# barathanaslan/whisper-ipa

Hardware: AMD Instinct MI355X
Metric: audio-seconds/sec transcribed (whisper-small, 30s clips) (higher is better)
Workload: dtype bf16

## Files before the change

include/wipa.h:

```cpp
#ifndef WIPA_H
#define WIPA_H
#include <stddef.h>
#include <stdint.h>
#ifdef __cplusplus
extern "C" {
#endif

typedef void* wipa_stream_t;

enum { WIPA_F32 = 0, WIPA_BF16 = 1, WIPA_FP8_E4M3 = 2  };
enum { WIPA_OK = 0, WIPA_ERR_ARG = -1, WIPA_ERR_HIP = -2, WIPA_ERR_STATE = -3 };

#define WIPA_N_SAMPLES 480000
#define WIPA_N_FRAMES 3000
#define WIPA_N_FFT 400
#define WIPA_HOP 160
#define WIPA_HEAD_DIM 64

int wipa_version(void);
const char* wipa_last_error(void);

int wipa_stream_create(wipa_stream_t* out);
int wipa_stream_create_cu_limited(int n_cus, wipa_stream_t* out);
int wipa_stream_destroy(wipa_stream_t s);
// ... 127 lines not shown
    const int32_t* pos;
    float* slabs;
    int64_t kv_batch_stride, slab_stride;
    int32_t B, d, H, dtype;
    float eps, qk_scale;
} wipa_self_block_desc;
int wipa_decode_self_block(const wipa_self_block_desc* d, wipa_stream_t s);
typedef struct wipa_cross_block_desc {
    const float* x_in;
    float* x_out;
    const float* slabs;
    const float* bias_o;
    const float* ln_w;
    const float* ln_b;
    const void* wq;
    const float* bq;
    const void* kv;
    void* out;
    int64_t slab_stride;
    int32_t n_slabs, B, d, H, Tk, dtype;
    float eps, qk_scale;
    int32_t cross_splits;
} wipa_cross_block_desc;
int wipa_decode_cross_block(const wipa_cross_block_desc* d, wipa_stream_t s);

int wipa_cross_absorbed_splits(int want, int Tk);
int wipa_cross_absorbed_resident_groups_for(int B, int d, int Tk, int n_splits, int64_t budget_bytes);
int wipa_cross_absorbed_resident_groups(int B, int d, int Tk, int n_splits);
size_t wipa_cross_absorbed_scratch_bytes(int B, int d, int Tk);
int wipa_cross_absorbed_init(int d);
int wipa_cross_absorbed_attention(const void* q, int64_t q_row_stride, const void* wkT, const void* xa, const void* wv, const float* bv,
                                  void* out, int64_t out_row_stride, void* scratch, size_t scratch_bytes, int B, int H, int d, int Tk,
                                  float k_scale, int n_splits, wipa_stream_t s);
int wipa_decode_cross_absorbed_block(const wipa_cross_block_desc* c, const void* wkT, const void* wv, const float* bv, void* scratch,
                                     size_t scratch_bytes, wipa_stream_t s);
int wipa_decode_cross_absorbed_block_out(const wipa_cross_block_desc* c, const void* wkT, const void* wv, const float* bv, const void* wo,
                                         const float* bo, float* slabs_out, int64_t slab_stride, void* scratch, size_t scratch_bytes,
                                         wipa_stream_t s);
int wipa_cross_absorbed_stream(const void* xa, void* scratch, size_t scratch_bytes, int B, int H, int d, int Tk, int n_splits,
                               wipa_stream_t s);

int wipa_greedy_step(const float* logits, int64_t ldl, int B, int V, const float* mask_first,
                     const float* mask_always, int32_t* tokens, int64_t ld_tok, const int32_t* pos_dev, int n_init,
                     int eot, float* sum_logprobs, int32_t* not_done, wipa_stream_t s);
int wipa_add_i32(int32_t* p, int32_t v, wipa_stream_t s);
int wipa_greedy_step_embed(const float* logits, int64_t ldl, int B, int V, const float* mask_first, const float* mask_always,
                           int32_t* tokens, int64_t ld_tok, int32_t* pos_dev, int64_t* posd_dev, int32_t* done_counter, int n_init,
                           int eot, float* sum_logprobs, int32_t* not_done, const void* tok_emb, int emb_dtype,
                           const float* emb_scale, const float* pos_emb, int n_ctx, float* x, const float* ln_w, const float* ln_b,
                           void* y, int y_dtype, int D, float eps, wipa_stream_t s);
#define WIPA_GREEDY_PARTS 2048
int wipa_logits_greedy_supported(int B, int V, int d, int dtype);
size_t wipa_logits_greedy_partials_bytes(int B);
int wipa_logits_greedy(const void* x, int64_t ldx, const void* w, int64_t ldw, float* logits, int64_t ldl, int B, int V, int d,
                       const float* mask_first, const float* mask_always, const int32_t* pos_dev, int n_init, float* partials,
                       size_t partials_bytes, wipa_stream_t s);
int wipa_greedy_step_embed_partials(const float* partials, int n_parts, int B, int32_t* tokens, int64_t ld_tok, int32_t* pos_dev,
                                    int64_t* posd_dev, int32_t* done_counter, int n_init, int eot, float* sum_logprobs,
                                    int32_t* not_done, const void* tok_emb, int emb_dtype, const float* emb_scale, const float* pos_emb,
                                    int n_ctx, float* x, const float* ln_w, const float* ln_b, void* y, int y_dtype, int D, float eps,
                                    wipa_stream_t s);
int wipa_embed_layernorm(const int32_t* tokens, int64_t ld_tok, int B, const int32_t* pos_dev, const void* tok_emb, int emb_dtype,
                         const float* emb_scale, const float* pos_emb, int n_ctx, float* x, const float* ln_w, const float* ln_b,
                         void* y, int y_dtype, int D, float eps, wipa_stream_t s);

typedef struct wipa_bpe wipa_bpe;
// ... 95 lines not shown
```

whisper_ipa_amd/_lib.py:

```python
from __future__ import annotations

import ctypes as C
import os
import threading

_HERE = os.path.dirname(os.path.abspath(__file__))
LIB_PATH = os.path.join(_HERE, "libwipa.so")

WIPA_F32, WIPA_BF16, WIPA_FP8_E4M3 = 0, 1, 2
GREEDY_PARTS = 2048
RESAMPLE_TILE = 512
ENC_GLOBAL, ENC_PER_LAYER = 7, 14
DEC_GLOBAL, DEC_PER_LAYER, DEC_FP8_PER_LAYER = 4, 20, 6
GEMM_DISPATCH = ("tile128", "tile256", "tile384", "tile384n", "tile256p", "skinny", "skinny_fp8", "skinny_ln", "kmajor", "split_k",
                 "tile_fp8", "tile_fp8_384")
ENC_FP8_PER_LAYER = 8
DEC_ABSORBED_PER_LAYER = 1

c_void_p, c_int, c_int64, c_size_t, c_float = C.c_void_p, C.c_int, C.c_int64, C.c_size_t, C.c_float


class GemmDesc(C.Structure):
    _fields_ = [
        ("A", c_void_p), ("W", c_void_p), ("C", c_void_p), ("bias", c_void_p), ("residual", c_void_p),
# ... 73 lines not shown
    "wipa_stream_destroy": (c_int, [c_void_p]),
    "wipa_resample_pad": (c_int, [c_void_p, c_size_t, c_void_p, _P(PcmClipDesc), c_int, c_void_p, c_size_t, c_void_p, c_void_p]),
    "wipa_logmel_tables_bytes": (c_size_t, [c_int]),
    "wipa_logmel_init": (c_int, [c_void_p, c_int, c_void_p]),
    "wipa_logmel_workspace_bytes": (c_size_t, [c_int, c_int]),
    "wipa_logmel": (c_int, [c_void_p, c_int, c_int, c_void_p, c_void_p, c_int, c_void_p, c_size_t, c_void_p]),
    "wipa_mel_pad_cast": (c_int, [c_void_p, c_int, c_int, c_void_p, c_int, c_void_p]),
    "wipa_gemm": (c_int, [_P(GemmDesc), c_void_p]),
    "wipa_gemm_dispatch_counts": (c_int, [_P(c_int64), c_int, c_int]),
    "wipa_layernorm": (c_int, [c_void_p, c_int, c_int64, c_void_p, c_int, c_int64, c_void_p, c_void_p, c_int, c_int,
                               c_float, c_void_p]),
    "wipa_layernorm_fp8": (c_int, [c_void_p, c_int64, c_void_p, c_int64, c_void_p, c_void_p, c_void_p, c_int, c_int, c_float, c_void_p]),
    "wipa_rowquant_fp8": (c_int, [c_void_p, c_int, c_int64, c_void_p, c_int64, c_void_p, c_int, c_int, c_void_p]),
    "wipa_add_slabs_layernorm": (c_int, [c_void_p, c_int64, c_void_p, c_int, c_int64, c_void_p, c_int, c_int64, c_void_p,
                                         c_void_p, c_int, c_int, c_float, c_void_p]),
    "wipa_embed_tokens": (c_int, [c_void_p, c_int64, c_int, c_int, c_int, c_void_p, c_void_p, c_int, c_void_p, c_void_p, c_void_p,
                                  c_int, c_void_p]),
    "wipa_attention": (c_int, [_P(AttnDesc), c_void_p]),
    "wipa_flash_attn_enc_f32": (c_int, [c_void_p, c_int64, c_void_p, c_int64, c_void_p, c_int64, c_void_p, c_int64, c_int, c_int,
                                       c_int, c_int, c_void_p]),
    "wipa_flash_attn_enc_bf16": (c_int, [c_void_p, c_int64, c_void_p, c_int64, c_void_p, c_int64, c_int, c_int, c_int,
                                         c_void_p]),
    "wipa_decode_attn": (c_int, [_P(AttnDesc), c_void_p]),
    "wipa_decode_cross_attn": (c_int, [c_void_p, c_void_p, c_void_p, c_int, c_int, c_int, c_int, c_void_p]),
    "wipa_decode_self_block": (c_int, [_P(SelfBlockDesc), c_void_p]),
    "wipa_decode_cross_block": (c_int, [_P(CrossBlockDesc), c_void_p]),
    "wipa_cross_absorbed_splits": (c_int, [c_int, c_int]),
    "wipa_cross_absorbed_resident_groups_for": (c_int, [c_int, c_int, c_int, c_int, c_int64]),
    "wipa_cross_absorbed_resident_groups": (c_int, [c_int, c_int, c_int, c_int]),
    "wipa_cross_absorbed_scratch_bytes": (c_size_t, [c_int, c_int, c_int]),
    "wipa_cross_absorbed_init": (c_int, [c_int]),
    "wipa_cross_absorbed_attention": (c_int, [c_void_p, c_int64, c_void_p, c_void_p, c_void_p, c_void_p, c_void_p, c_int64, c_void_p, c_size_t,
                                              c_int, c_int, c_int, c_int, c_float, c_int, c_void_p]),
    "wipa_cross_absorbed_stream": (c_int, [c_void_p, c_void_p, c_size_t, c_int, c_int, c_int, c_int, c_int, c_void_p]),
    "wipa_decode_cross_absorbed_block": (c_int, [_P(CrossBlockDesc), c_void_p, c_void_p, c_void_p, c_void_p, c_size_t, c_void_p]),
    "wipa_decode_cross_absorbed_block_out": (c_int, [_P(CrossBlockDesc), c_void_p, c_void_p, c_void_p, c_void_p, c_void_p, c_void_p, c_int64,
                                                     c_void_p, c_size_t, c_void_p]),
    "wipa_greedy_step": (c_int, [c_void_p, c_int64, c_int, c_int, c_void_p, c_void_p, c_void_p, c_int64, c_void_p, c_int,
                                 c_int, c_void_p, c_void_p, c_void_p]),
    "wipa_add_i32": (c_int, [c_void_p, C.c_int32, c_void_p]),
    "wipa_greedy_step_embed": (c_int, [c_void_p, c_int64, c_int, c_int, c_void_p, c_void_p, c_void_p, c_int64, c_void_p, c_void_p, c_void_p,
                                       c_int, c_int, c_void_p, c_void_p, c_void_p, c_int, c_void_p, c_void_p, c_int, c_void_p, c_void_p,
                                       c_void_p, c_void_p, c_int, c_int, c_float, c_void_p]),
    "wipa_logits_greedy_supported": (c_int, [c_int, c_int, c_int, c_int]),
    "wipa_logits_greedy_partials_bytes": (c_size_t, [c_int]),
    "wipa_logits_greedy": (c_int, [c_void_p, c_int64, c_void_p, c_int64, c_void_p, c_int64, c_int, c_int, c_int, c_void_p, c_void_p, c_void_p,
                                   c_int, c_void_p, c_size_t, c_void_p]),
    "wipa_greedy_step_embed_partials": (c_int, [c_void_p, c_int, c_int, c_void_p, c_int64, c_void_p, c_void_p, c_void_p, c_int, c_int, c_void_p,
                                                c_void_p, c_void_p, c_int, c_void_p, c_void_p, c_int, c_void_p, c_void_p, c_void_p, c_void_p,
                                                c_int, c_int, c_float, c_void_p]),
    "wipa_embed_layernorm": (c_int, [c_void_p, c_int64, c_int, c_void_p, c_void_p, c_int, c_void_p, c_void_p, c_int, c_void_p, c_void_p,
                                     c_void_p, c_void_p, c_int, c_int, c_float, c_void_p]),
    "wipa_bpe_create": (c_void_p, [c_void_p, c_void_p, c_void_p, c_int]),
    "wipa_bpe_free": (None, [c_void_p]),
    "wipa_bpe_encode_piece": (c_int, [c_void_p, C.c_char_p, c_int, c_void_p, c_int]),
    "wipa_bpe_decode": (c_int, [c_void_p, c_void_p, c_int, c_void_p, c_int]),
    "wipa_build_token_batch": (c_int, [c_void_p, c_void_p, c_int, c_void_p, c_int, C.c_int32, c_void_p, c_int64]),
    "wipa_profile_begin": (c_int, [c_void_p]),
    "wipa_profile_end": (c_int, [_P(c_float), _P(c_int)]),
    "wipa_encoder_workspace_bytes": (c_size_t, [_P(ModelCfg), c_int]),
    "wipa_encoder_forward": (c_int, [_P(ModelCfg), _P(c_void_p), c_void_p, c_void_p, c_void_p, c_size_t, c_int, c_void_p]),
    "wipa_decoder_layout": (c_int, [_P(ModelCfg), c_int, _P(DecLayout)]),
    "wipa_decoder_set_audio": (c_int, [_P(ModelCfg), _P(c_void_p), c_void_p, c_void_p, c_size_t, c_int, c_void_p]),
    "wipa_decoder_begin": (c_int, [_P(ModelCfg), c_void_p, c_size_t, c_int, _P(C.c_int32), c_int, c_void_p]),
    "wipa_decoder_run": (c_int, [_P(ModelCfg), _P(c_void_p), c_void_p, c_size_t, c_int, c_int, c_int, c_void_p, c_void_p, c_int,
                                 c_int, c_void_p]),
# ... 58 lines not shown
```

whisper_ipa_amd/csrc/cross_absorbed.hip:

```cpp
#include <cstdlib>
#include <mutex>
#include <type_traits>

#include "attn_stream.h"
#include "wipa_common.h"

namespace {

constexpr int FT = 32;
constexpr long long XA_RESIDENT_MB_SHARED = 16;
constexpr long long XA_RESIDENT_MB_LONE = -1;
typedef __attribute__((address_space(3))) void* lds_ptr_a;
typedef int v2i32 __attribute__((ext_vector_type(2)));

struct AbsParams {
    const __bf16* qp;
    const __bf16* xa;
    float* part_m;
    float* part_l;
    float* part_o;
    int Tk, n_splits, tiles_per_split, H;
    int resident_groups;
};

constexpr int POLICY_DEFAULT = 0, POLICY_NT = 2;

__device__ __forceinline__ int swz(int row) { return (row & 7) << 1; }

template <int D>
struct AbsCfg {
    static constexpr int NW = 4;
    static constexpr int ROWB = D * 2;
    static constexpr int TILE = FT * ROWB;
    static constexpr int SX = NW * 2 * 64 * 4 * (int)sizeof(float);
    static constexpr int NBUF = (3 * TILE + SX <= 160 * 1024) ? 3 : 2;
    static constexpr int SMEM = NBUF * TILE + SX;
};

template <int D>
__global__ __launch_bounds__(512, 1) void cross_absorbed_kernel(AbsParams p) {
    typedef AbsCfg<D> X;
    constexpr int NW = X::NW, ROWB = X::ROWB, TILE = X::TILE, NBUF = X::NBUF;
    constexpr int NDMA = TILE / 1024 / NW;
    constexpr int KS = D / NW / 32;
    constexpr int CT = D / NW / 16;
    static_assert(D % (32 * NW) == 0 && TILE % (1024 * NW) == 0, "width");
    extern __shared__ __attribute__((aligned(1024))) char smem[];
    float* sx = reinterpret_cast<float*>(smem + NBUF * TILE);
    const int tid = threadIdx.x, lane = tid & 63;
    const int wave = __builtin_amdgcn_readfirstlane(tid >> 6);
    const int l15 = lane & 15, g = lane >> 4;
    const int split = blockIdx.x, b = blockIdx.y;
    const int tile0 = split * p.tiles_per_split;
    const int n_tiles_total = (p.Tk + FT - 1) / FT;
    const int nt = max(0, min(p.tiles_per_split, n_tiles_total - tile0));
    const __bf16* xb = p.xa + (int64_t)b * p.Tk * D;

    bf16x8 qf[KS];
    {
        const __bf16* qr = p.qp + ((int64_t)b * 16 + l15) * D + wave * (D / NW) + 8 * g;
#pragma unroll
        for (int ks = 0; ks < KS; ++ks) qf[ks] = *reinterpret_cast<const bf16x8*>(qr + 32 * ks);
    }
    const __amdgpu_buffer_rsrc_t rX = __builtin_amdgcn_make_buffer_rsrc((void*)xb, 0, 0x7fffffff, 0x00020000);
    int drow[NDMA], dch[NDMA];
#pragma unroll
    for (int i = 0; i < NDMA; ++i) {
        const int off = 1024 * (NDMA * wave + i) + 16 * lane;
        drow[i] = off / ROWB;
        dch[i] = ((off % ROWB) >> 4) ^ swz(off / ROWB);
    }
    const int res_tiles = p.resident_groups / 2;
    auto stage_as = [&](auto policy, int t, int buf) {
        constexpr int AUX = decltype(policy)::value;
        const int f0 = (tile0 + t) * FT;
#pragma unroll
        for (int i = 0; i < NDMA; ++i) {
            const int voff = min(f0 + drow[i], p.Tk - 1) * ROWB + dch[i] * 16;
            __builtin_amdgcn_raw_ptr_buffer_load_lds(rX, (lds_ptr_a)(smem + buf * TILE + 1024 * (NDMA * wave + i)), 16, voff, 0, 0, AUX);
        }
    };
    auto stage = [&](int t, int buf) {
        if (t < res_tiles) stage_as(std::integral_constant<int, POLICY_DEFAULT>{}, t, buf);
        else stage_as(std::integral_constant<int, POLICY_NT>{}, t, buf);
    };
    auto wait_dma = [&](bool one_behind) {
        if (one_behind) {
            if constexpr (NDMA == 12) asm volatile("s_waitcnt vmcnt(12)" ::: "memory");
            else if constexpr (NDMA == 16) asm volatile("s_waitcnt vmcnt(16)" ::: "memory");
// ... 136 lines not shown
        p.part_m[ps * 16 + l15] = m_run;
        p.part_l[ps * 16 + l15] = l_run;
    }
    float* po = p.part_o + ps * 16 * D;
#pragma unroll
    for (int c = 0; c < CT; ++c)
#pragma unroll
        for (int r = 0; r < 4; ++r) po[(int64_t)(4 * g + r) * D + wave * (D / NW) + 16 * c + l15] = acc[c][r];
}

typedef __bf16 bf16x4v __attribute__((ext_vector_type(4)));

template <int D, int NW_>
struct AbsCfg2 {
    static constexpr int NWV = NW_;
    static constexpr int GF = 16;
    static constexpr int ROWB = D * 2;
    static constexpr int SLOT = GF * ROWB;
    static constexpr int SMEM_LOOP = NWV * 2 * SLOT;
    static constexpr int MROW = D + 4;
    static constexpr int SMEM_MERGE = NWV * 16 * MROW * 4 + NWV * 32 * 4;
    static constexpr int SMEM = SMEM_LOOP > SMEM_MERGE ? SMEM_LOOP : SMEM_MERGE;
};

#define WIPA_TR8(X, A, IMM)                                                                                                          \
    asm volatile("ds_read_b64_tr_b16 %0, %8 offset:" #IMM "\n\tds_read_b64_tr_b16 %1, %9 offset:" #IMM                              \
                 "\n\tds_read_b64_tr_b16 %2, %10 offset:" #IMM "\n\tds_read_b64_tr_b16 %3, %11 offset:" #IMM                          \
                 "\n\tds_read_b64_tr_b16 %4, %12 offset:" #IMM "\n\tds_read_b64_tr_b16 %5, %13 offset:" #IMM                          \
                 "\n\tds_read_b64_tr_b16 %6, %14 offset:" #IMM "\n\tds_read_b64_tr_b16 %7, %15 offset:" #IMM "\n\ts_waitcnt lgkmcnt(0)" \
                 : "=&v"(X[0]), "=&v"(X[1]), "=&v"(X[2]), "=&v"(X[3]), "=&v"(X[4]), "=&v"(X[5]), "=&v"(X[6]), "=&v"(X[7])           \
                 : "v"(A[0]), "v"(A[1]), "v"(A[2]), "v"(A[3]), "v"(A[4]), "v"(A[5]), "v"(A[6]), "v"(A[7])                           \
                 : "memory")

template <int D, int NW_>
__global__ __launch_bounds__(64 * NW_, 1) void cross_absorbed_v2_kernel(AbsParams p) {
    typedef AbsCfg2<D, NW_> X;
    constexpr int NWV = X::NWV, GF = X::GF, ROWB = X::ROWB, SLOT = X::SLOT;
    constexpr int NDMA = SLOT / 1024;
    constexpr int KS = D / 32;
    constexpr int CT = D / 16;
    static_assert(SLOT % 1024 == 0 && NDMA <= 32 && CT % 8 == 0 && KS % 4 == 0 && CT / 8 <= 8 && D % 128 == 0, "width");
    extern __shared__ __attribute__((aligned(1024))) char smem[];
    const int tid = threadIdx.x, lane = tid & 63;
    const int wave = __builtin_amdgcn_readfirstlane(tid >> 6);
    const int l15 = lane & 15, g = lane >> 4;
    const int split = blockIdx.x, b = blockIdx.y;
    const int groups_total = (p.Tk + GF - 1) / GF;
    const int gps = 2 * p.tiles_per_split;
    const int g0 = split * gps;
    const int ng = max(0, min(gps, groups_total - g0));
    const int my_n = ng > wave ? (ng - wave + NWV - 1) / NWV : 0;
    const __bf16* xb = p.xa + (int64_t)b * p.Tk * D;
    char* my = smem + wave * (2 * SLOT);

    bf16x8 qf[KS];
    {
        const __bf16* qr = p.qp + ((int64_t)b * 16 + l15) * D + 8 * g;
#pragma unroll
        for (int ks = 0; ks < KS; ++ks) qf[ks] = *reinterpret_cast<const bf16x8*>(qr + 32 * ks);
    }
    const __amdgpu_buffer_rsrc_t rX = __builtin_amdgcn_make_buffer_rsrc((void*)xb, 0, 0x7fffffff, 0x00020000);
    constexpr int G1K = (ROWB % 1024 == 0) ? 1024 : ((ROWB % 512 == 0) ? 512 : 256);
    constexpr int PER = ROWB / G1K, QR = 1024 / G1K;
    static_assert(NDMA % PER == 0 && PER <= 3 && (QR == 1 || QR == 2 || QR == 4), "transfer / row period");
    int dma_a[PER], dma_b[PER];
#pragma unroll
    for (int t = 0; t < PER; ++t) {
        const int off = 1024 * t + 16 * lane;
        const int r = off / ROWB, c = (off - r * ROWB) >> 4;
        dma_a[t] = (c ^ (r << 1)) << 4;
        dma_b[t] = r * ROWB;
    }
    int lane_v = lane;
    auto stage_as = [&](auto policy, int i_local, int slot) {
        constexpr int AUX = decltype(policy)::value;
        const int f0 = (g0 + wave + NWV * i_local) * GF;
        if (f0 + GF <= p.Tk) {
#pragma unroll
            for (int i = 0; i < NDMA; ++i) {
                const int j = i / PER, t = i % PER;
                const int sj = (((QR * j) & 7) << 1) << 4;
                const int voff = (dma_a[t] ^ sj) + dma_b[t];
                __builtin_amdgcn_raw_ptr_buffer_load_lds(rX, (lds_ptr_a)(my + slot * SLOT + 1024 * i), 16, voff, (f0 + QR * j) * ROWB, 0, AUX);
            }
        } else {
// ... 472 lines not shown
    __syncthreads();
#pragma unroll
    for (int i = 0; i < CG / 8; ++i) {
        const int e = tid + 512 * i, row = e >> 6, j = e & 63;
        float q = 0.f;
#pragma unroll
        for (int w = 0; w < 8; ++w) q += red[w][row][j];
        qh[row][j] = (__bf16)((q + p.bq[h * 64 + j]) * p.q_scale);
    }
    if constexpr (CG < 16) {
        for (int e = tid; e < (16 - CG) * 64; e += 512) qh[CG + (e >> 6)][e & 63] = (__bf16)0.f;
    }
    __syncthreads();
    {
        const bf16x8 a0 = *reinterpret_cast<const bf16x8*>(&qh[l15][8 * g]);
        const bf16x8 a1 = *reinterpret_cast<const bf16x8*>(&qh[l15][32 + 8 * g]);
#pragma unroll
        for (int i = 0; i < NTW; ++i) {
            const int nt = wave * NTW + i;
            if (nt < NT) {
                f32x4 acc = {0.f, 0.f, 0.f, 0.f};
                acc = __builtin_amdgcn_mfma_f32_16x16x32_bf16(a0, wkf[i][0], acc, 0, 0, 0);
                acc = __builtin_amdgcn_mfma_f32_16x16x32_bf16(a1, wkf[i][1], acc, 0, 0, 0);
#pragma unroll
                for (int r = 0; r < 4; ++r) {
                    const int bb_ = b0 + 4 * g + r;
                    if (4 * g + r < CG && bb_ < p.B) p.qp[((int64_t)bb_ * 16 + h) * D + 16 * nt + l15] = (__bf16)(acc[r] * p.k_scale);
                }
            }
        }
    }
}

template <int D>
int launch_attn(const AbsParams& p_in, int B, hipStream_t s) {
    const char* e = getenv("WIPA_ABS_KERNEL");
    AbsParams p = p_in;
    p.resident_groups = wipa_cross_absorbed_resident_groups(B, D, p.Tk, p.n_splits);
    if ((e && atoi(e) == 1) || (D > 768 && !(e && atoi(e) == 2)))
        hipLaunchKernelGGL((cross_absorbed_kernel<D>), dim3(p.n_splits, B), dim3(64 * AbsCfg<D>::NW), AbsCfg<D>::SMEM, s, p);
    else if constexpr (D > 768)
        hipLaunchKernelGGL((cross_absorbed_v2_kernel<D, 2>), dim3(p.n_splits, B), dim3(128), (AbsCfg2<D, 2>::SMEM), s, p);
    else {
        static const int waves = [] { const char* w = getenv("WIPA_ABS_WAVES"); return w ? atoi(w) : 3; }();
        if (waves == 2) hipLaunchKernelGGL((cross_absorbed_v2_kernel<D, 2>), dim3(p.n_splits, B), dim3(128), (AbsCfg2<D, 2>::SMEM), s, p);
        else hipLaunchKernelGGL((cross_absorbed_v2_kernel<D, 3>), dim3(p.n_splits, B), dim3(192), (AbsCfg2<D, 3>::SMEM), s, p);
    }
    return WIPA_OK;
}

AbsParams abs_params(void* scratch, int B, int d, int Tk, int S, int H, const void* xa) {
    char* sc = (char*)scratch;
    AbsParams p = {};
    p.qp = (const __bf16*)sc; p.xa = (const __bf16*)xa;
    p.part_m = (float*)(sc + (size_t)B * 16 * d * 2);
    p.part_l = p.part_m + (size_t)B * S * 16;
    p.part_o = p.part_l + (size_t)B * S * 16;
    p.Tk = Tk; p.n_splits = S; p.H = H;
    const int tiles = (Tk + FT - 1) / FT;
    p.tiles_per_split = (tiles + S - 1) / S;
    return p;
}

template <typename F>
int for_width(int d, F f) {
    if (d == 384) return f(std::integral_constant<int, 384>());
    if (d == 512) return f(std::integral_constant<int, 512>());
    if (d == 768) return f(std::integral_constant<int, 768>());
    if (d == 1024) return f(std::integral_constant<int, 1024>());
    return WIPA_ERR_ARG;
}

}

extern "C" int wipa_cross_absorbed_splits(int want, int Tk) {
    const int tiles = (Tk + FT - 1) / FT;
    static const int dflt = [] { const char* e = getenv("WIPA_ABS_SPLITS"); const int v = e ? atoi(e) : 4; return (v >= 1 && v <= 4) ? v : 4; }();
    int s = (want >= 1 && want <= 4) ? want : dflt;
    if (s > tiles / 2) s = tiles / 2;
    return s < 1 ? 1 : s;
}
// ... 1 lines not shown
extern "C" int wipa_cross_absorbed_resident_groups_for(int B, int d, int Tk, int n_splits, int64_t budget_bytes) {
    if (B < 1 || d < 1 || Tk < 1) return 0;
    const int S = wipa_cross_absorbed_splits(n_splits, Tk);
    const int tiles = (Tk + FT - 1) / FT;
    const int gps = 2 * ((tiles + S - 1) / S);
    if (budget_bytes < 0 || budget_bytes >= (int64_t)B * Tk * d * 2) return gps;
    const int64_t g = budget_bytes / ((int64_t)B * S * 16 * d * 2);
    return g < gps ? (int)g : gps;
}

extern "C" int wipa_cross_absorbed_resident_groups(int B, int d, int Tk, int n_splits) {
    static const int64_t env_mb = [] { const char* e = getenv("WIPA_XA_RESIDENT_MB"); return e ? (int64_t)atoll(e) : (int64_t)INT64_MIN; }();
    const int S = wipa_cross_absorbed_splits(n_splits, Tk);
    int64_t mb = env_mb;
    if (mb == INT64_MIN) mb = (S <= 2) ? XA_RESIDENT_MB_SHARED : XA_RESIDENT_MB_LONE;
    return wipa_cross_absorbed_resident_groups_for(B, d, Tk, S, mb < 0 ? -1 : mb * 1000000);
}

extern "C" size_t wipa_cross_absorbed_scratch_bytes(int B, int d, int Tk) {
    (void)Tk;
    return (size_t)B * 16 * d * 2 + (size_t)B * 4 * 16 * (2 + (size_t)d) * 4 + 1024;
}

extern "C" int wipa_cross_absorbed_init(int d) {
    static std::mutex mu;
    static bool done[4] = {false, false, false, false};
    const int wi = d == 384 ? 0 : d == 512 ? 1 : d == 768 ? 2 : d == 1024 ? 3 : -1;
    if (wi < 0) return WIPA_ERR_ARG;
    std::lock_guard<std::mutex> lk(mu);
    if (done[wi]) return WIPA_OK;
    hipError_t e = hipSuccess;
    for_width(d, [&](auto width) {
        constexpr int D = decltype(width)::value;
        e = hipFuncSetAttribute(reinterpret_cast<const void*>(&cross_absorbed_kernel<D>), hipFuncAttributeMaxDynamicSharedMemorySize,
                                AbsCfg<D>::SMEM);
        if constexpr (D <= 768) {
            if (e == hipSuccess)
                e = hipFuncSetAttribute(reinterpret_cast<const void*>(&cross_absorbed_v2_kernel<D, 3>),
                                        hipFuncAttributeMaxDynamicSharedMemorySize, AbsCfg2<D, 3>::SMEM);
        }
        if (e == hipSuccess)
            e = hipFuncSetAttribute(reinterpret_cast<const void*>(&cross_absorbed_v2_kernel<D, 2>),
                                    hipFuncAttributeMaxDynamicSharedMemorySize, AbsCfg2<D, 2>::SMEM);
        return WIPA_OK;
    });
    WIPA_CHECK_HIP(e);
    done[wi] = true;
    return WIPA_OK;
}

extern "C" int wipa_cross_absorbed_stream(const void* xa, void* scratch, size_t scratch_bytes, int B, int H, int d, int Tk, int n_splits,
                                          wipa_stream_t stream) {
    WIPA_REQUIRE(xa && scratch && B > 0 && H >= 1 && H <= 16 && d == H * 64 && (d == 384 || d == 512 || d == 768 || d == 1024) && Tk >= 1 &&
                     n_splits >= 0 && n_splits <= 4,
                 "wipa_cross_absorbed_stream: bad arguments");
    WIPA_REQUIRE(scratch_bytes >= wipa_cross_absorbed_scratch_bytes(B, d, Tk), "wipa_cross_absorbed_stream: scratch too small");
    const int rc0 = wipa_cross_absorbed_init(d);
    if (rc0 != WIPA_OK) return rc0;
    const int S = wipa_cross_absorbed_splits(n_splits, Tk);
    const AbsParams p = abs_params(scratch, B, d, Tk, S, H, xa);
    const int rc = for_width(d, [&](auto width) { return launch_attn<decltype(width)::value>(p, B, (hipStream_t)stream); });
    if (rc != WIPA_OK) return rc;
    WIPA_LAUNCH_CHECK();
    return WIPA_OK;
}

extern "C" int wipa_cross_absorbed_attention(const void* q, int64_t q_row_stride, const void* wkT, const void* xa, const void* wv,
                                             const float* bv, void* out, int64_t out_row_stride, void* scratch, size_t scratch_bytes,
                                             int B, int H, int d, int Tk, float k_scale, int n_splits, wipa_stream_t stream) {
    WIPA_REQUIRE(q && wkT && xa && wv && bv && out && scratch, "wipa_cross_absorbed_attention: null pointer");
    WIPA_REQUIRE(n_splits >= 0 && n_splits <= 4, "wipa_cross_absorbed_attention: n_splits %d (0 = default, 1..4)", n_splits);
    WIPA_REQUIRE(B > 0 && B <= 65535 && H >= 1 && H <= 16 && d == H * 64 && (d == 384 || d == 512 || d == 768 || d == 1024) && Tk >= 1,
                 "wipa_cross_absorbed_attention: bf16, <= 16 heads of 64, d in {384, 512, 768, 1024} (got H=%d d=%d)", H, d);
    WIPA_REQUIRE(q_row_stride % 8 == 0 && out_row_stride >= d && ((uintptr_t)q % 16) == 0 && ((uintptr_t)xa % 16) == 0 &&
                     ((uintptr_t)wkT % 16) == 0 && ((uintptr_t)wv % 16) == 0 && ((uintptr_t)scratch % 16) == 0,
                 "wipa_cross_absorbed_attention: operands must be 16-byte aligned");
    WIPA_REQUIRE((int64_t)Tk * d * 2 < ((int64_t)1 << 31), "wipa_cross_absorbed_attention: clip too long for 32-bit tile offsets");
    WIPA_REQUIRE(scratch_bytes >= wipa_cross_absorbed_scratch_bytes(B, d, Tk), "wipa_cross_absorbed_attention: scratch too small");
    hipStream_t s = (hipStream_t)stream;
    {
        const int rc0 = wipa_cross_absorbed_init(d);
        if (rc0 != WIPA_OK) return rc0;
    }
    const int S = wipa_cross_absorbed_splits(n_splits, Tk);
    const AbsParams p = abs_params(scratch, B, d, Tk, S, H, xa);
    const dim3 gq(16, (B + 15) / 16, 4), gm(H, (B + WIPA_MERGE_CL - 1) / WIPA_MERGE_CL);
    const char* st_env = getenv("WIPA_ABS_STAGES");
    const int stages = st_env ? atoi(st_env) : 7;
    const int rc = for_width(d, [&](auto width) {
        constexpr int D = decltype(width)::value;
        int rc = WIPA_OK;
        if (stages & 1)
            hipLaunchKernelGGL((cross_absorb_q_kernel<D>), gq, dim3(64), 0, s, (const __bf16*)q, q_row_stride, (const __bf16*)wkT,
                               const_cast<__bf16*>(p.qp), B, H, k_scale);
        if (stages & 2) rc = launch_attn<D>(p, B, s);
        if (rc == WIPA_OK && (stages & 4))
            hipLaunchKernelGGL((cross_merge_proj_kernel<D>), gm, dim3(64 * MergeCfg<D>::NWM), 0, s, p.part_m, p.part_l, p.part_o, S,
                               (const __bf16*)wv, bv, (__bf16*)out, out_row_stride, B);
        return rc;
    });
    if (rc != WIPA_OK) return rc;
    WIPA_LAUNCH_CHECK();
    return WIPA_OK;
}

static int absorbed_block(const wipa_cross_block_desc* c, const void* wkT, const void* wv, const float* bv, const void* wo, const float* bo,
                          float* slabs_out, int64_t slab_stride, void* scratch, size_t scratch_bytes, wipa_stream_t stream);

extern "C" int wipa_decode_cross_absorbed_block(const wipa_cross_block_desc* c, const void* wkT, const void* wv, const float* bv, void* scratch,
                                                size_t scratch_bytes, wipa_stream_t stream) {
    WIPA_REQUIRE(c && c->out, "wipa_decode_cross_absorbed_block: null pointer");
    return absorbed_block(c, wkT, wv, bv, nullptr, nullptr, nullptr, 0, scratch, scratch_bytes, stream);
}

extern "C" int wipa_decode_cross_absorbed_block_out(const wipa_cross_block_desc* c, const void* wkT, const void* wv, const float* bv,
                                                    const void* wo, const float* bo, float* slabs_out, int64_t slab_stride, void* scratch,
                                                    size_t scratch_bytes, wipa_stream_t stream) {
    WIPA_REQUIRE(c && wo && bo && slabs_out && slab_stride >= (int64_t)c->B * c->d && ((uintptr_t)wo % 16) == 0,
                 "wipa_decode_cross_absorbed_block_out: null pointer / short slab stride");
    return absorbed_block(c, wkT, wv, bv, wo, bo, slabs_out, slab_stride, scratch, scratch_bytes, stream);
}

static int absorbed_block(const wipa_cross_block_desc* c, const void* wkT, const void* wv, const float* bv, const void* wo, const float* bo,
                          float* slabs_out, int64_t slab_stride, void* scratch, size_t scratch_bytes, wipa_stream_t stream) {
    WIPA_REQUIRE(c && c->x_in && c->x_out && c->ln_w && c->ln_b && c->wq && c->bq && c->kv && (c->out || wo) && wkT && wv && bv && scratch,
                 "wipa_decode_cross_absorbed_block: null pointer");
    WIPA_REQUIRE(c->x_in != c->x_out, "wipa_decode_cross_absorbed_block: x_out must not alias x_in");
    const int B = c->B, H = c->H, d = c->d, Tk = c->Tk;
// ... 36 lines not shown
```

whisper_ipa_amd/csrc/runtime.hip:

```cpp
#include <algorithm>
#include <cstdarg>
#include <cstdlib>
#include <cstring>
#include <strings.h>
#include <map>
#include <mutex>
#include <tuple>
#include <vector>

#include "wipa_common.h"

static thread_local char g_err[512] = "";
void wipa_set_error(const char* fmt, ...) {
    va_list ap;
    va_start(ap, fmt);
    vsnprintf(g_err, sizeof(g_err), fmt, ap);
    va_end(ap);
}
extern "C" const char* wipa_last_error(void) { return g_err; }
extern "C" int wipa_version(void) { return 100; }

extern "C" int wipa_stream_create_cu_limited(int n_cus, wipa_stream_t* out) {
    int dev = 0, total = 0;
    WIPA_CHECK_HIP(hipGetDevice(&dev));
// ... 254 lines not shown
        }
    }
    PROF(PROF_NORM, wipa_layernorm(x, WIPA_F32, d, out, dt, d, (const float*)w[5], (const float*)w[6], M, d, 1e-5f, stream));
    return WIPA_OK;
}

namespace {

constexpr int MAX_SLABS = 4;
struct DecScratch {
    size_t x, x2, ln, q, ao, h, slabs, posd, absorbed, greedy_part, total;
};
inline int k_slices_for(int K, int dtype) {
    const int ksteps = K * (int)wipa_dtype_size(dtype) / 64;
    int s = ksteps / 12;
    return s < 1 ? 1 : (s > MAX_SLABS ? MAX_SLABS : s);
}
int decode_mode(const wipa_model_cfg* cfg, int B);
constexpr int MAX_PROMPT = 4;
DecScratch dec_scratch(const wipa_model_cfg* c, int B) {
    const size_t e = wipa_dtype_size(c->dtype), d = c->n_text_state;
    const size_t R = (size_t)B * MAX_PROMPT;
    DecScratch s;
    size_t o = 0;
    s.x = o;    o += align256(R * d * 4);
    s.x2 = o;   o += align256((size_t)B * d * 4);
    s.ln = o;   o += align256(R * d * e);
    s.q = o;    o += align256(R * d * e);
    s.ao = o;   o += align256(R * d * e);
    s.h = o;    o += align256(R * 4 * d * e);
    s.slabs = o; o += align256(std::max((size_t)MAX_SLABS * R, (size_t)c->n_text_head * B) * d * 4);
    s.posd = o; o += 256;
    s.absorbed = o;
    if (c->dec_cross_absorbed) o += align256(wipa_cross_absorbed_scratch_bytes(B, (int)d, c->n_audio_ctx));
    s.greedy_part = o;
    if (wipa_logits_greedy_supported(B, c->n_vocab, (int)d, c->dtype)) o += align256(wipa_logits_greedy_partials_bytes(B));
    s.total = o;
    return s;
}

wipa_dec_layout dec_layout(const wipa_model_cfg* c, int B) {
    const size_t e = wipa_dtype_size(c->dtype);
    const size_t d = c->n_text_state, H = c->n_text_head;
    wipa_dec_layout L;
    size_t o = 0;
    L.ld_tok = c->n_text_ctx + 8;
    L.tokens = o; o += align256((size_t)B * L.ld_tok * 4);
    L.pos = o; o += 256;
    L.not_done = o; o += 256;
    L.sum_logprobs = o; o += align256((size_t)B * 4);
    L.ld_logits = round_up(c->n_vocab, 8);
    L.logits = o; o += align256((size_t)B * L.ld_logits * 4);
    L.cross_kv = o; o += align256(c->dec_cross_absorbed ? (size_t)B * c->n_audio_ctx * d * e
                                                        : (size_t)c->n_text_layer * B * 2 * H * c->n_audio_ctx * 64 * e);
    L.self_kv = o; o += align256((size_t)c->n_text_layer * 3 * B * c->n_text_ctx * d * e);
    L.scratch = o; o += dec_scratch(c, B).total;
    L.total_bytes = o;
    return L;
}

__global__ void advance_pos_kernel(int32_t* pos, int64_t* posd, int d) {
    const int p = *pos + 1;
    *pos = p;
    *posd = (int64_t)p * d;
}

__global__ void fill_tokens_kernel(int32_t* tokens, int64_t ld_tok, int B, int n_init, int i0, int i1, int i2, int i3,
                                   const int32_t* extra) {
    const int b = blockIdx.x * blockDim.x + threadIdx.x;
    if (b >= B) return;
    const int first4[4] = {i0, i1, i2, i3};
    for (int t = 0; t < n_init; ++t) tokens[(int64_t)b * ld_tok + t] = (t < 4 || !extra) ? first4[t & 3] : extra[t];
}

bool absorbed_block_fused() {
    const char* e = getenv("WIPA_ABS_FUSED_PROLOGUE");
    return !(e && atoi(e) == 0);
}

bool absorbed_merge_out() {
    const char* e = getenv("WIPA_ABS_MERGE_OUT");
    return e && atoi(e) == 1;
}
bool tail_fused() {
    const char* e = getenv("WIPA_DECODE_TAIL");
    return !(e && atoi(e) == 0);
}
thread_local bool t_lean_logits = false;
bool logits_fused(const wipa_model_cfg* cfg, int B) {
    const char* e = getenv("WIPA_LOGITS_FUSED");
    const bool on = !(e && atoi(e) == 0);
    return on && tail_fused() && cfg->dec_w_dtype == 0 && wipa_logits_greedy_supported(B, cfg->n_vocab, cfg->n_text_state, cfg->dtype);
}
int32_t* done_counter_of(char* st, const wipa_dec_layout& L) { return (int32_t*)(st + L.pos + 64); }

int enqueue_step_head(const wipa_model_cfg* cfg, const void* const* w, char* st, const wipa_dec_layout& L, int B, wipa_stream_t stream) {
    const DecScratch S = dec_scratch(cfg, B);
    char* sc = st + L.scratch;
    const void* const* lw0 = w + WIPA_DEC_GLOBAL;
    return wipa_embed_layernorm((const int32_t*)(st + L.tokens), L.ld_tok, B, (const int32_t*)(st + L.pos), w[0], emb_dtype(cfg), emb_scale(cfg, w),
                                (const float*)w[1], cfg->n_text_ctx, (float*)(sc + S.x), (const float*)lw0[0], (const float*)lw0[1], sc + S.ln,
                                cfg->dtype, cfg->n_text_state, 1e-5f, stream);
}

int enqueue_step(const wipa_model_cfg* cfg, const void* const* w, char* st, const wipa_dec_layout& L, int B, int n_init,
                 int eot, const float* mask_first, const float* mask_always, wipa_stream_t stream) {
    const int dt = cfg->dtype;
    const bool tail = tail_fused();
    const size_t e = wipa_dtype_size(dt);
    const int d = cfg->n_text_state, H = cfg->n_text_head, nctx = cfg->n_text_ctx, Ta = cfg->n_audio_ctx;
    const DecScratch S = dec_scratch(cfg, B);
    char* sc = st + L.scratch;
    float* x = (float*)(sc + S.x);
    float* x_other = (float*)(sc + S.x2);
    const bool absorbed = cfg->dec_cross_absorbed != 0;
// ... 261 lines not shown
        RT_CALL(ln_step(lw[0], lw[1]));
        {
            wipa_gemm_desc g;
            memset(&g, 0, sizeof(g));
        g.stream_weights = 1;
            g.col_scale_n = 2 * d; g.col_scale = QK_SCALE;
            g.rg_in = P; g.rg_valid = P; g.rg_stride = (int64_t)nctx * d;
            g.cg_in = d; g.cg_stride = (int64_t)B * nctx * d;
            RT_CALL(gemm(ln, d, lw[2], d, skv, d, M, 3 * d, d, dt, dt, (const float*)lw[3], 0, nullptr, stream, &g));
        }
        {
            wipa_attn_desc a;
            memset(&a, 0, sizeof(a));
            const size_t slot = (size_t)B * nctx * d * e;
            a.q = skv; a.k = skv + slot; a.v = skv + 2 * slot; a.out = ao;
            a.q_bs = (int64_t)nctx * d; a.q_rs = d; a.q_hs = 64;
            a.k_bs = a.q_bs; a.k_rs = d; a.k_hs = 64;
            a.v_bs = a.q_bs; a.v_rs = d; a.v_hs = 64;
            a.o_bs = (int64_t)P * d; a.o_rs = d; a.o_hs = 64;
            a.B = B; a.H = H; a.Tq = P; a.Tk = P; a.causal = 1; a.dtype = dt;
            RT_CALL(wipa_attention(&a, stream));
        }
        RT_CALL(residual_gemm(ao, d, lw[4], lw[5]));
        RT_CALL(ln_step(lw[6], lw[7]));
        {
            wipa_gemm_desc g;
            memset(&g, 0, sizeof(g));
        g.stream_weights = 1;
            g.col_scale_n = d; g.col_scale = QK_SCALE;
            RT_CALL(gemm(ln, d, lw[8], d, q, d, M, d, d, dt, dt, (const float*)lw[9], 0, nullptr, stream, &g));
        }
        if (cfg->dec_cross_absorbed) {
            const void* wkT = w[WIPA_DEC_GLOBAL + WIPA_DEC_PER_LAYER * cfg->n_text_layer + WIPA_DEC_ABSORBED_PER_LAYER * l];
            for (int t = 0; t < P; ++t)
                RT_CALL(wipa_cross_absorbed_attention((const char*)q + (size_t)t * d * e, (int64_t)P * d, wkT, st + L.cross_kv,
                                                      (const char*)lw[10] + (size_t)d * d * e, (const float*)lw[11] + d,
                                                      (char*)ao + (size_t)t * d * e, (int64_t)P * d, sc + S.absorbed, S.greedy_part - S.absorbed, B,
                                                      H, d, Ta, QK_SCALE, cfg->dec_cross_splits, stream));
        } else {
            RT_CALL(wipa_decode_cross_attn_multi(q, ckv, ao, B, H, Ta, P, dt, stream));
        }
        RT_CALL(residual_gemm(ao, d, lw[12], lw[13]));
        RT_CALL(ln_step(lw[14], lw[15]));
        {
            wipa_gemm_desc g;
            memset(&g, 0, sizeof(g));
            g.stream_weights = 1;
            RT_CALL(gemm(ln, d, lw[16], d, hb, 4 * d, M, 4 * d, d, dt, dt, (const float*)lw[17], 1, nullptr, stream, &g));
        }
        RT_CALL(residual_gemm(hb, 4 * d, lw[18], lw[19]));
    }
    RT_CALL(ln_step(w[2], w[3]));
    float* logits = (float*)(st + L.logits);
    RT_CALL(gemm(ln + (size_t)(P - 1) * d * e, (int64_t)P * d, w[0], d, logits, L.ld_logits, B, cfg->n_vocab, d, dt, WIPA_F32, nullptr, 0,
                 nullptr, stream));
    hipLaunchKernelGGL(set_pos_kernel, dim3(1), dim3(1), 0, (hipStream_t)stream, pos, posd, P - 1, d);
    RT_CALL(wipa_greedy_step(logits, L.ld_logits, B, cfg->n_vocab, mask_first, mask_always, tokens, L.ld_tok, pos, n_init,
                             eot, (float*)(st + L.sum_logprobs), (int32_t*)(st + L.not_done), stream));
    hipLaunchKernelGGL(advance_pos_kernel, dim3(1), dim3(1), 0, (hipStream_t)stream, pos, posd, d);
    WIPA_LAUNCH_CHECK();
    return WIPA_OK;
}

bool counters_attached() {
    const char* e = getenv("ROCPROF_COUNTER_COLLECTION");
    return e && *e && strcmp(e, "0") != 0 && strcasecmp(e, "false") != 0;
}
bool graphs_allowed() {
    const char* g = getenv("WIPA_DECODE_GRAPH");
    if (g && (strcmp(g, "0") == 0 || strcasecmp(g, "off") == 0)) return false;
    if (g && strcasecmp(g, "force") == 0) return true;
// ... 177 lines not shown
        *out = exec;
        return WIPA_OK;
    };
    hipGraphExec_t full = nullptr, lean = nullptr;
    RT_CALL(step_graph(false, &full));
    if (lean_ok && n_steps > 1) RT_CALL(step_graph(true, &lean));
    for (int i = 0; i < n_steps; ++i) WIPA_CHECK_HIP(hipGraphLaunch((lean && i + 1 < n_steps) ? lean : full, s));
    return WIPA_OK;
}

extern "C" int wipa_decoder_prefill(const wipa_model_cfg* cfg, const void* const* w, void* state, size_t state_bytes, int B,
                                    int n_init, int eot, const float* mask_first, const float* mask_always, int use_graph,
                                    wipa_stream_t stream) {
    RT_CALL(cfg_check(cfg));
    SplitScope split_scope(cfg);
    WIPA_REQUIRE(w && state && mask_first && mask_always && B > 0, "wipa_decoder_prefill: bad arguments");
    WIPA_REQUIRE(n_init >= 1 && n_init <= MAX_PROMPT, "wipa_decoder_prefill: 1..%d prompt tokens (got %d)", MAX_PROMPT, n_init);
    W8Scope w8_scope(cfg, w);
    const wipa_dec_layout L = dec_layout(cfg, B);
    RT_CALL(state_fits("wipa_decoder_prefill", L, state_bytes));
    char* st = (char*)state;
    auto enqueue = [&]() -> int {
        if (n_init == 1) {
            if (step_needs_head(cfg, B)) RT_CALL(enqueue_step_head(cfg, w, st, L, B, stream));
            return enqueue_decode_step(cfg, w, st, L, B, n_init, eot, mask_first, mask_always, stream);
        }
        return enqueue_prefill(cfg, w, st, L, B, n_init, eot, mask_first, mask_always, stream);
    };
    hipStream_t s = (hipStream_t)stream;
    RT_CALL(init_before_capture(cfg));
    WIPA_CHECK_HIP(hipMemsetAsync(done_counter_of(st, L), 0, sizeof(int32_t), s));
    if (!use_graph || s == nullptr || !graphs_allowed()) return enqueue();
    hipGraphExec_t exec = nullptr;
    const GraphKey key(state, (const void*)w, (const void*)mask_first, (const void*)mask_always, B, n_init, eot, cfg->dtype * 2 + t_f32_split + 4 * decode_mode(cfg, B) + 16 * cfg->dec_w_dtype + 64 * cfg->dec_cross_absorbed * (absorbed_block_fused() ? 2 : 1) + 256 * (int)tail_fused() + 512 * (int)absorbed_merge_out() + 1024 * cfg->dec_cross_splits + 8192 * (int)(!use_fused_step(cfg, B) && logits_fused(cfg, B)), cfg->weights_generation, 1);
    {
        std::lock_guard<std::mutex> lk(g_graph_mu);
        auto it = g_graphs.find(key);
        if (it != g_graphs.end()) exec = it->second;
    }
    if (!exec) {
        hipGraph_t graph = nullptr;
        WIPA_CHECK_HIP(hipStreamBeginCapture(s, hipStreamCaptureModeRelaxed));
        const int rc = enqueue();
        const hipError_t ee = hipStreamEndCapture(s, &graph);
        if (rc != WIPA_OK) {
            if (graph) hipGraphDestroy(graph);
            return rc;
        }
        WIPA_CHECK_HIP(ee);
        WIPA_CHECK_HIP(hipGraphInstantiate(&exec, graph, nullptr, nullptr, 0));
        WIPA_CHECK_HIP(hipGraphDestroy(graph));
        std::lock_guard<std::mutex> lk(g_graph_mu);
        g_graphs[key] = exec;
    }
    WIPA_CHECK_HIP(hipGraphLaunch(exec, s));
    return WIPA_OK;
}

extern "C" int wipa_decoder_release(void* state) {
    std::lock_guard<std::mutex> lk(g_graph_mu);
    for (auto it = g_graphs.begin(); it != g_graphs.end();) {
        if (std::get<0>(it->first) == state) {
            hipGraphExecDestroy(it->second);
            it = g_graphs.erase(it);
        } else {
            ++it;
        }
// ... 108 lines not shown
```

Baseline: 26880.

## Batch prefill cross-attention rows into one absorbed-attention launch

Prefill used to call the absorbed cross-attention once per prompt position, which meant P separate launches of the q-absorb, attention and merge kernels. The new rows variant handles all B*P query rows in a single launch. Each row indexes its clip's audio features, and a workgroup mapping interleaves rows that share the same clip and split so they run close together and reuse the same xa tile in cache. The cost is a larger scratch allocation sized for all rows and more template instantiations. An environment flag, on by default, controls the path.

```diff
diff --git a/include/wipa.h b/include/wipa.h
--- a/include/wipa.h
+++ b/include/wipa.h
@@ -183,6 +183,9 @@
 int wipa_cross_absorbed_attention(const void* q, int64_t q_row_stride, const void* wkT, const void* xa, const void* wv, const float* bv,
                                   void* out, int64_t out_row_stride, void* scratch, size_t scratch_bytes, int B, int H, int d, int Tk,
                                   float k_scale, int n_splits, wipa_stream_t s);
+int wipa_cross_absorbed_attention_rows(const void* q, int64_t q_row_stride, const void* wkT, const void* xa, const void* wv, const float* bv,
+                                       void* out, int64_t out_row_stride, void* scratch, size_t scratch_bytes, int B, int R, int H, int d,
+                                       int Tk, float k_scale, int n_splits, wipa_stream_t s);
 int wipa_decode_cross_absorbed_block(const wipa_cross_block_desc* c, const void* wkT, const void* wv, const float* bv, void* scratch,
                                      size_t scratch_bytes, wipa_stream_t s);
 int wipa_decode_cross_absorbed_block_out(const wipa_cross_block_desc* c, const void* wkT, const void* wv, const float* bv, const void* wo,
diff --git a/whisper_ipa_amd/_lib.py b/whisper_ipa_amd/_lib.py
--- a/whisper_ipa_amd/_lib.py
+++ b/whisper_ipa_amd/_lib.py
@@ -129,6 +129,8 @@
     "wipa_cross_absorbed_init": (c_int, [c_int]),
     "wipa_cross_absorbed_attention": (c_int, [c_void_p, c_int64, c_void_p, c_void_p, c_void_p, c_void_p, c_void_p, c_int64, c_void_p, c_size_t,
                                               c_int, c_int, c_int, c_int, c_float, c_int, c_void_p]),
+    "wipa_cross_absorbed_attention_rows": (c_int, [c_void_p, c_int64, c_void_p, c_void_p, c_void_p, c_void_p, c_void_p, c_int64, c_void_p,
+                                                   c_size_t, c_int, c_int, c_int, c_int, c_int, c_float, c_int, c_void_p]),
     "wipa_cross_absorbed_stream": (c_int, [c_void_p, c_void_p, c_size_t, c_int, c_int, c_int, c_int, c_int, c_void_p]),
     "wipa_decode_cross_absorbed_block": (c_int, [_P(CrossBlockDesc), c_void_p, c_void_p, c_void_p, c_void_p, c_size_t, c_void_p]),
     "wipa_decode_cross_absorbed_block_out": (c_int, [_P(CrossBlockDesc), c_void_p, c_void_p, c_void_p, c_void_p, c_void_p, c_void_p, c_int64,
diff --git a/whisper_ipa_amd/csrc/cross_absorbed.hip b/whisper_ipa_amd/csrc/cross_absorbed.hip
--- a/whisper_ipa_amd/csrc/cross_absorbed.hip
+++ b/whisper_ipa_amd/csrc/cross_absorbed.hip
@@ -21,7 +21,34 @@
     float* part_o;
     int Tk, n_splits, tiles_per_split, H;
     int resident_groups;
+    int rows_per_xa;
 };
+
+template <bool ROWS>
+__device__ __forceinline__ void abs_workgroup(const AbsParams& p, int& split, int& row, int& clip) {
+    if constexpr (!ROWS) {
+        split = blockIdx.x;
+        row = clip = blockIdx.y;
+    } else {
+        const int R = p.rows_per_xa, S = p.n_splits;
+        const int L = blockIdx.x + gridDim.x * blockIdx.y;
+        const int n_streams = gridDim.x * gridDim.y / R;
+        const int full = n_streams & ~7;
+        int u, j;
+        if (L < full * R) {
+            const int k = L / (8 * R), in = L - k * (8 * R);
+            u = 8 * k + (in & 7);
+            j = in >> 3;
+        } else {
+            const int lt = L - full * R, nt = n_streams - full;
+            j = lt / nt;
+            u = full + (lt - j * nt);
+        }
+        clip = u / S;
+        split = u - clip * S;
+        row = clip * R + j;
+    }
+}
 
 constexpr int POLICY_DEFAULT = 0, POLICY_NT = 2;
 
@@ -37,7 +64,7 @@
     static constexpr int SMEM = NBUF * TILE + SX;
 };
 
-template <int D>
+template <int D, bool ROWS = false>
 __global__ __launch_bounds__(512, 1) void cross_absorbed_kernel(AbsParams p) {
     typedef AbsCfg<D> X;
     constexpr int NW = X::NW, ROWB = X::ROWB, TILE = X::TILE, NBUF = X::NBUF;
@@ -50,11 +77,12 @@
     const int tid = threadIdx.x, lane = tid & 63;
     const int wave = __builtin_amdgcn_readfirstlane(tid >> 6);
     const int l15 = lane & 15, g = lane >> 4;
-    const int split = blockIdx.x, b = blockIdx.y;
+    int split, b, clip;
+    abs_workgroup<ROWS>(p, split, b, clip);
     const int tile0 = split * p.tiles_per_split;
     const int n_tiles_total = (p.Tk + FT - 1) / FT;
     const int nt = max(0, min(p.tiles_per_split, n_tiles_total - tile0));
-    const __bf16* xb = p.xa + (int64_t)b * p.Tk * D;
+    const __bf16* xb = p.xa + (int64_t)clip * p.Tk * D;
 
     bf16x8 qf[KS];
     {
@@ -257,7 +285,7 @@
                  : "v"(A[0]), "v"(A[1]), "v"(A[2]), "v"(A[3]), "v"(A[4]), "v"(A[5]), "v"(A[6]), "v"(A[7])                           \
                  : "memory")
 
-template <int D, int NW_>
+template <int D, int NW_, bool ROWS = false>
 __global__ __launch_bounds__(64 * NW_, 1) void cross_absorbed_v2_kernel(AbsParams p) {
     typedef AbsCfg2<D, NW_> X;
     constexpr int NWV = X::NWV, GF = X::GF, ROWB = X::ROWB, SLOT = X::SLOT;
@@ -269,13 +297,14 @@
     const int tid = threadIdx.x, lane = tid & 63;
     const int wave = __builtin_amdgcn_readfirstlane(tid >> 6);
     const int l15 = lane & 15, g = lane >> 4;
-    const int split = blockIdx.x, b = blockIdx.y;
+    int split, b, clip;
+    abs_workgroup<ROWS>(p, split, b, clip);
     const int groups_total = (p.Tk + GF - 1) / GF;
     const int gps = 2 * p.tiles_per_split;
     const int g0 = split * gps;
     const int ng = max(0, min(gps, groups_total - g0));
     const int my_n = ng > wave ? (ng - wave + NWV - 1) / NWV : 0;
-    const __bf16* xb = p.xa + (int64_t)b * p.Tk * D;
+    const __bf16* xb = p.xa + (int64_t)clip * p.Tk * D;
     char* my = smem + wave * (2 * SLOT);
 
     bf16x8 qf[KS];
@@ -814,21 +843,28 @@
     }
 }
 
-template <int D>
-int launch_attn(const AbsParams& p_in, int B, hipStream_t s) {
+template <int D, bool ROWS>
+int launch_attn_as(const AbsParams& p_in, int B, int R, hipStream_t s) {
     const char* e = getenv("WIPA_ABS_KERNEL");
     AbsParams p = p_in;
+    p.rows_per_xa = R;
     p.resident_groups = wipa_cross_absorbed_resident_groups(B, D, p.Tk, p.n_splits);
+    B *= R;
     if ((e && atoi(e) == 1) || (D > 768 && !(e && atoi(e) == 2)))
-        hipLaunchKernelGGL((cross_absorbed_kernel<D>), dim3(p.n_splits, B), dim3(64 * AbsCfg<D>::NW), AbsCfg<D>::SMEM, s, p);
+        hipLaunchKernelGGL((cross_absorbed_kernel<D, ROWS>), dim3(p.n_splits, B), dim3(64 * AbsCfg<D>::NW), AbsCfg<D>::SMEM, s, p);
     else if constexpr (D > 768)
-        hipLaunchKernelGGL((cross_absorbed_v2_kernel<D, 2>), dim3(p.n_splits, B), dim3(128), (AbsCfg2<D, 2>::SMEM), s, p);
+        hipLaunchKernelGGL((cross_absorbed_v2_kernel<D, 2, ROWS>), dim3(p.n_splits, B), dim3(128), (AbsCfg2<D, 2>::SMEM), s, p);
     else {
         static const int waves = [] { const char* w = getenv("WIPA_ABS_WAVES"); return w ? atoi(w) : 3; }();
-        if (waves == 2) hipLaunchKernelGGL((cross_absorbed_v2_kernel<D, 2>), dim3(p.n_splits, B), dim3(128), (AbsCfg2<D, 2>::SMEM), s, p);
-        else hipLaunchKernelGGL((cross_absorbed_v2_kernel<D, 3>), dim3(p.n_splits, B), dim3(192), (AbsCfg2<D, 3>::SMEM), s, p);
+        if (waves == 2) hipLaunchKernelGGL((cross_absorbed_v2_kernel<D, 2, ROWS>), dim3(p.n_splits, B), dim3(128), (AbsCfg2<D, 2>::SMEM), s, p);
+        else hipLaunchKernelGGL((cross_absorbed_v2_kernel<D, 3, ROWS>), dim3(p.n_splits, B), dim3(192), (AbsCfg2<D, 3>::SMEM), s, p);
     }
     return WIPA_OK;
+}
+
+template <int D>
+int launch_attn(const AbsParams& p, int B, hipStream_t s, int R = 1) {
+    return R == 1 ? launch_attn_as<D, false>(p, B, 1, s) : launch_attn_as<D, true>(p, B, R, s);
 }
 
 AbsParams abs_params(void* scratch, int B, int d, int Tk, int S, int H, const void* xa) {
@@ -896,16 +932,22 @@
     hipError_t e = hipSuccess;
     for_width(d, [&](auto width) {
         constexpr int D = decltype(width)::value;
-        e = hipFuncSetAttribute(reinterpret_cast<const void*>(&cross_absorbed_kernel<D>), hipFuncAttributeMaxDynamicSharedMemorySize,
-                                AbsCfg<D>::SMEM);
-        if constexpr (D <= 768) {
+        auto raise = [&](auto rows) {
+            constexpr bool ROWS = decltype(rows)::value;
             if (e == hipSuccess)
-                e = hipFuncSetAttribute(reinterpret_cast<const void*>(&cross_absorbed_v2_kernel<D, 3>),
-                                        hipFuncAttributeMaxDynamicSharedMemorySize, AbsCfg2<D, 3>::SMEM);
-        }
-        if (e == hipSuccess)
-            e = hipFuncSetAttribute(reinterpret_cast<const void*>(&cross_absorbed_v2_kernel<D, 2>),
-                                    hipFuncAttributeMaxDynamicSharedMemorySize, AbsCfg2<D, 2>::SMEM);
+                e = hipFuncSetAttribute(reinterpret_cast<const void*>(&cross_absorbed_kernel<D, ROWS>),
+                                        hipFuncAttributeMaxDynamicSharedMemorySize, AbsCfg<D>::SMEM);
+            if constexpr (D <= 768) {
+                if (e == hipSuccess)
+                    e = hipFuncSetAttribute(reinterpret_cast<const void*>(&cross_absorbed_v2_kernel<D, 3, ROWS>),
+                                            hipFuncAttributeMaxDynamicSharedMemorySize, AbsCfg2<D, 3>::SMEM);
+            }
+            if (e == hipSuccess)
+                e = hipFuncSetAttribute(reinterpret_cast<const void*>(&cross_absorbed_v2_kernel<D, 2, ROWS>),
+                                        hipFuncAttributeMaxDynamicSharedMemorySize, AbsCfg2<D, 2>::SMEM);
+        };
+        raise(std::false_type{});
+        raise(std::true_type{});
         return WIPA_OK;
     });
     WIPA_CHECK_HIP(e);
@@ -932,8 +974,18 @@
 extern "C" int wipa_cross_absorbed_attention(const void* q, int64_t q_row_stride, const void* wkT, const void* xa, const void* wv,
                                              const float* bv, void* out, int64_t out_row_stride, void* scratch, size_t scratch_bytes,
                                              int B, int H, int d, int Tk, float k_scale, int n_splits, wipa_stream_t stream) {
+    return wipa_cross_absorbed_attention_rows(q, q_row_stride, wkT, xa, wv, bv, out, out_row_stride, scratch, scratch_bytes, B, 1, H, d, Tk,
+                                              k_scale, n_splits, stream);
+}
+
+extern "C" int wipa_cross_absorbed_attention_rows(const void* q, int64_t q_row_stride, const void* wkT, const void* xa, const void* wv,
+                                                  const float* bv, void* out, int64_t out_row_stride, void* scratch, size_t scratch_bytes,
+                                                  int B, int R, int H, int d, int Tk, float k_scale, int n_splits, wipa_stream_t stream) {
     WIPA_REQUIRE(q && wkT && xa && wv && bv && out && scratch, "wipa_cross_absorbed_attention: null pointer");
     WIPA_REQUIRE(n_splits >= 0 && n_splits <= 4, "wipa_cross_absorbed_attention: n_splits %d (0 = default, 1..4)", n_splits);
+    WIPA_REQUIRE(B > 0 && R >= 1 && (int64_t)B * R <= 65535, "wipa_cross_absorbed_attention: B %d x R %d rows (1..65535)", B, R);
+    const int n_xa = B;
+    B *= R;
     WIPA_REQUIRE(B > 0 && B <= 65535 && H >= 1 && H <= 16 && d == H * 64 && (d == 384 || d == 512 || d == 768 || d == 1024) && Tk >= 1,
                  "wipa_cross_absorbed_attention: bf16, <= 16 heads of 64, d in {384, 512, 768, 1024} (got H=%d d=%d)", H, d);
     WIPA_REQUIRE(q_row_stride % 8 == 0 && out_row_stride >= d && ((uintptr_t)q % 16) == 0 && ((uintptr_t)xa % 16) == 0 &&
@@ -957,7 +1009,7 @@
         if (stages & 1)
             hipLaunchKernelGGL((cross_absorb_q_kernel<D>), gq, dim3(64), 0, s, (const __bf16*)q, q_row_stride, (const __bf16*)wkT,
                                const_cast<__bf16*>(p.qp), B, H, k_scale);
-        if (stages & 2) rc = launch_attn<D>(p, B, s);
+        if (stages & 2) rc = launch_attn<D>(p, n_xa, s, R);
         if (rc == WIPA_OK && (stages & 4))
             hipLaunchKernelGGL((cross_merge_proj_kernel<D>), gm, dim3(64 * MergeCfg<D>::NWM), 0, s, p.part_m, p.part_l, p.part_o, S,
                                (const __bf16*)wv, bv, (__bf16*)out, out_row_stride, B);
diff --git a/whisper_ipa_amd/csrc/runtime.hip b/whisper_ipa_amd/csrc/runtime.hip
--- a/whisper_ipa_amd/csrc/runtime.hip
+++ b/whisper_ipa_amd/csrc/runtime.hip
@@ -310,7 +310,7 @@
     s.slabs = o; o += align256(std::max((size_t)MAX_SLABS * R, (size_t)c->n_text_head * B) * d * 4);
     s.posd = o; o += 256;
     s.absorbed = o;
-    if (c->dec_cross_absorbed) o += align256(wipa_cross_absorbed_scratch_bytes(B, (int)d, c->n_audio_ctx));
+    if (c->dec_cross_absorbed) o += align256(wipa_cross_absorbed_scratch_bytes((int)R, (int)d, c->n_audio_ctx));
     s.greedy_part = o;
     if (wipa_logits_greedy_supported(B, c->n_vocab, (int)d, c->dtype)) o += align256(wipa_logits_greedy_partials_bytes(B));
     s.total = o;
@@ -359,6 +359,10 @@
 bool absorbed_merge_out() {
     const char* e = getenv("WIPA_ABS_MERGE_OUT");
     return e && atoi(e) == 1;
+}
+bool prefill_rows() {
+    const char* e = getenv("WIPA_PREFILL_ROWS");
+    return !(e && atoi(e) == 0);
 }
 bool tail_fused() {
     const char* e = getenv("WIPA_DECODE_TAIL");
@@ -686,11 +690,17 @@
         }
         if (cfg->dec_cross_absorbed) {
             const void* wkT = w[WIPA_DEC_GLOBAL + WIPA_DEC_PER_LAYER * cfg->n_text_layer + WIPA_DEC_ABSORBED_PER_LAYER * l];
-            for (int t = 0; t < P; ++t)
-                RT_CALL(wipa_cross_absorbed_attention((const char*)q + (size_t)t * d * e, (int64_t)P * d, wkT, st + L.cross_kv,
-                                                      (const char*)lw[10] + (size_t)d * d * e, (const float*)lw[11] + d,
-                                                      (char*)ao + (size_t)t * d * e, (int64_t)P * d, sc + S.absorbed, S.greedy_part - S.absorbed, B,
-                                                      H, d, Ta, QK_SCALE, cfg->dec_cross_splits, stream));
+            if (prefill_rows()) {
+                RT_CALL(wipa_cross_absorbed_attention_rows(q, d, wkT, st + L.cross_kv, (const char*)lw[10] + (size_t)d * d * e,
+                                                           (const float*)lw[11] + d, ao, d, sc + S.absorbed, S.greedy_part - S.absorbed, B, P, H,
+                                                           d, Ta, QK_SCALE, cfg->dec_cross_splits, stream));
+            } else {
+                for (int t = 0; t < P; ++t)
+                    RT_CALL(wipa_cross_absorbed_attention((const char*)q + (size_t)t * d * e, (int64_t)P * d, wkT, st + L.cross_kv,
+                                                          (const char*)lw[10] + (size_t)d * d * e, (const float*)lw[11] + d,
+                                                          (char*)ao + (size_t)t * d * e, (int64_t)P * d, sc + S.absorbed,
+                                                          S.greedy_part - S.absorbed, B, H, d, Ta, QK_SCALE, cfg->dec_cross_splits, stream));
+            }
         } else {
             RT_CALL(wipa_decode_cross_attn_multi(q, ckv, ao, B, H, Ta, P, dt, stream));
         }
@@ -934,7 +944,7 @@
     WIPA_CHECK_HIP(hipMemsetAsync(done_counter_of(st, L), 0, sizeof(int32_t), s));
     if (!use_graph || s == nullptr || !graphs_allowed()) return enqueue();
     hipGraphExec_t exec = nullptr;
-    const GraphKey key(state, (const void*)w, (const void*)mask_first, (const void*)mask_always, B, n_init, eot, cfg->dtype * 2 + t_f32_split + 4 * decode_mode(cfg, B) + 16 * cfg->dec_w_dtype + 64 * cfg->dec_cross_absorbed * (absorbed_block_fused() ? 2 : 1) + 256 * (int)tail_fused() + 512 * (int)absorbed_merge_out() + 1024 * cfg->dec_cross_splits + 8192 * (int)(!use_fused_step(cfg, B) && logits_fused(cfg, B)), cfg->weights_generation, 1);
+    const GraphKey key(state, (const void*)w, (const void*)mask_first, (const void*)mask_always, B, n_init, eot, cfg->dtype * 2 + t_f32_split + 4 * decode_mode(cfg, B) + 16 * cfg->dec_w_dtype + 64 * cfg->dec_cross_absorbed * (absorbed_block_fused() ? 2 : 1) + 256 * (int)tail_fused() + 512 * (int)absorbed_merge_out() + 1024 * cfg->dec_cross_splits + 8192 * (int)(!use_fused_step(cfg, B) && logits_fused(cfg, B)) + 16384 * (int)prefill_rows(), cfg->weights_generation, 1);
     {
         std::lock_guard<std::mutex> lk(g_graph_mu);
         auto it = g_graphs.find(key);
```

Result: no change. 27060, median of 6 (+0.7%).
